# DavidSlayback/po-brax

Measured on AMD Instinct MI355X. Metric: env-steps/sec AntHeavenHell batch 65536 @1/2/4/8 GPU; % HBM roofline, higher is better.
Workload: dtype f32

## Files before the change

### po-brax_amd/csrc/pob_blockwalk.h

```cpp
#pragma once
#include <stdint.h>
#ifdef POB_BW_HOST
#define POB_BW_D static inline
#else
#define POB_BW_D __device__ __forceinline__
#endif

#define QBW_WAVES 4
#define QBW_WCAP 50
#define QBW_SLOT_DW 11
#define QBW_CON_DW 5
#define QBW_LANE_MAX 64
#define QBW_CAP (QBW_WAVES * QBW_WCAP)
#define QBW_SEG_FLOATS (QBW_WCAP * QBW_SLOT_DW + 1)
#define QBW_NO_CONTACT (-1)

POB_BW_D constexpr int bw_item_off(const int j) { return QBW_SLOT_DW * j; }
POB_BW_D constexpr int bw_meta_off(const int j) { return QBW_SLOT_DW * j + 2 * QBW_CON_DW; }
POB_BW_D constexpr int bw_con_off(const int c) { return QBW_SLOT_DW * (c >> 1) + QBW_CON_DW * (c & 1); }
POB_BW_D constexpr int bw_count_off() { return QBW_WCAP * QBW_SLOT_DW; }

POB_BW_D constexpr int bw_meta(const int bit, const bool seg, const int slot) { return bit | (seg ? 64 : 0) | (slot << 7); }
POB_BW_D constexpr int bw_meta_bit(const int m) { return m & 63; }
POB_BW_D constexpr bool bw_meta_seg(const int m) { return (m & 64) != 0; }
POB_BW_D constexpr int bw_meta_slot(const int m) { return (m >> 7) & 3; }

POB_BW_D int bw_lane_count(const uint64_t m0, const uint64_t m1, const uint64_t m2) {
  const int n = __builtin_popcountll(m0) + __builtin_popcountll(m1) + __builtin_popcountll(m2);
  return n < QBW_LANE_MAX ? n : QBW_LANE_MAX;
}
POB_BW_D void bw_prefix_step(const uint64_t m, const int lane, const int b, int &base, int &tot) {
  base += __builtin_popcountll(m & ((1ull << lane) - 1ull)) << b;
  tot += __builtin_popcountll(m) << b;
}
#define QBW_PREFIX_BITS 7
#define QBW_PREFIX_SHORT_BITS 2
POB_BW_D constexpr bool bw_prefix_needs_all(const int count) { return count >= (1 << QBW_PREFIX_SHORT_BITS); }

POB_BW_D bool bw_next_item(uint64_t (&M)[3], int &slot, int &bit) {
  const bool h0 = M[0] != 0ull, h1 = M[1] != 0ull, h2 = M[2] != 0ull;
  const bool has = h0 | h1 | h2;
  slot = h0 ? 0 : (h1 ? 1 : 2);
  const uint64_t ml = h0 ? M[0] : (h1 ? M[1] : M[2]);
  bit = has ? __builtin_ctzll(ml) : 0;
  const uint64_t pop = has ? ml & (0ull - ml) : 0ull;
  M[0] = h0 ? M[0] & ~pop : M[0];
  M[1] = (!h0 & h1) ? M[1] & ~pop : M[1];
  M[2] = (!h0 & !h1) ? M[2] & ~pop : M[2];
  return has;
}

struct BwDeal {
  int off[QBW_WAVES];
  int T;
  bool ovf;
};
POB_BW_D BwDeal bw_deal(const int n0, const int n1, const int n2, const int n3, const int cap) {
  BwDeal d;
  d.off[0] = 0; d.off[1] = n0; d.off[2] = n0 + n1; d.off[3] = n0 + n1 + n2;
  const int T = n0 + n1 + n2 + n3;
  d.ovf = (T > cap) | (n0 > QBW_WCAP) | (n1 > QBW_WCAP) | (n2 > QBW_WCAP) | (n3 > QBW_WCAP);
  d.T = d.ovf ? 0 : T;
  return d;
}
POB_BW_D int bw_rounds(const BwDeal &d) { return (d.T + 7) >> 3; }
POB_BW_D int bw_first_round(const int w, const int sub) { return (w + sub) & (QBW_WAVES - 1); }
POB_BW_D void bw_item_owner(const BwDeal &d, const int i, int &w, int &j) {
  w = (i >= d.off[1] ? 1 : 0) + (i >= d.off[2] ? 1 : 0) + (i >= d.off[3] ? 1 : 0);
  j = i - (w == 0 ? 0 : (w == 1 ? d.off[1] : (w == 2 ? d.off[2] : d.off[3])));
}
POB_BW_D void bw_apply_range(const int base, const int n, const bool ovf, int &c0, int &c1) {
  c0 = 2 * base;
  c1 = ovf ? c0 : 2 * (base + n);
}
POB_BW_D void bw_body_ranges(const int base, const int n0, const int n1, const int n2, const bool ovf, int (&c)[4]) {
  c[0] = 2 * base;
  c[1] = ovf ? c[0] : c[0] + 2 * n0;
  c[2] = ovf ? c[0] : c[1] + 2 * n1;
  c[3] = ovf ? c[0] : c[2] + 2 * n2;
}

POB_BW_D constexpr bool bw_quad_lead(const int lane) { return (lane & 3) == 0; }
POB_BW_D constexpr int bw_quad_torso_count(const int lane, const int n0) { return bw_quad_lead(lane) ? n0 : 0; }
POB_BW_D void bw_quad_ranges(const int lane, const int base0, const int n0, const int base, const int n1, const int n2,
                             const bool ovf, int (&c)[5]) {
  c[0] = 2 * base0;
  c[1] = ovf ? c[0] : c[0] + 2 * n0;
  c[2] = 2 * (base + bw_quad_torso_count(lane, n0));
  c[3] = ovf ? c[2] : c[2] + 2 * n1;
  c[4] = ovf ? c[2] : c[3] + 2 * n2;
}

#define QBW_HIT_ITEMS 16
POB_BW_D constexpr uint32_t bw_hit_bits(const bool h0, const bool h1, const int i) {
  return ((h0 ? 1u : 0u) | (h1 ? 2u : 0u)) << (2 * i);
}
POB_BW_D constexpr int bw_hit_count(const int tot, const bool wide) { return wide && tot <= QBW_WCAP ? QBW_WCAP + 1 : tot; }
```

### po-brax_amd/csrc/pob_kernels.hip

```cpp
#include <hip/hip_fp16.h>
#include <hip/hip_runtime.h>

#include <climits>
#include <cstdio>
#include <cstdlib>
#include <cstring>
#include <mutex>
#include <new>
#include <type_traits>
#include <vector>

#include "../../include/pob.h"

#include "pob_quad.h"
#include "pob_octet.h"
#include "pob_hexa.h"
#include "pob_physics.h"

namespace pob {
void default_params(pob_params &p);
const char *build_system(int kind, const pob_params &p, pob_sys &s);
int gather_grid(const pob_params &p, float *xyz, int cap);
}

struct pob_env {
  pob_sys sys;
  pob_sys *d_sys = nullptr;
  pob_params params;
  float *d_grid = nullptr;
  uint32_t *d_scratch = nullptr;
  int device = 0;
  int n_cu = 256;
};

#define POB_MIXED (-1)
#define POB_F_STAGED (1u << 16)
#define POB_F_INT_FORCE_FIXUP (1u << 30)
#define POB_F_INT_BWCAP_SHIFT 20
#define POB_F_INT_BWCAP_MASK (0xFFu << POB_F_INT_BWCAP_SHIFT)
#define POB_F_INT_HITW_SHIFT 17
#define POB_F_INT_HITW_MASK (0x7u << POB_F_INT_HITW_SHIFT)
#define POB_F_INTERNAL (POB_F_STAGED | POB_F_INT_FORCE_FIXUP | POB_F_INT_BWCAP_MASK | POB_F_INT_HITW_MASK)
#define POB_F_PUBLIC (POB_F_EPISODE | POB_F_AUTORESET | POB_F_ZERO_STEPS_ON_DONE)

#define POB_STATE_FIELDS(X)                                                                    \
  X(pos) X(rot) X(vel) X(ang) X(obs) X(reward) X(done) X(steps) X(truncation) X(m0) X(m1) X(m2) \
  X(rng) X(first_pos) X(first_rot) X(first_vel) X(first_ang) X(first_obs) X(any_done) X(done_u8) X(trunc_i32) \
  X(m0_i32) X(m1_i32) X(any_done_clear) X(obs_masked) X(ovf_mark)

struct StatePtrs {
  float *pos, *rot, *vel, *ang, *obs, *reward, *done, *steps, *truncation, *m0, *m1, *m2;
  uint32_t *rng;
  float *first_pos, *first_rot, *first_vel, *first_ang, *first_obs;
  uint32_t *any_done;
  uint8_t *done_u8;
  int32_t *trunc_i32, *m0_i32, *m1_i32;
  uint32_t *any_done_clear;
  float *obs_masked;
  uint8_t *ovf_mark;
};
POB_D void store_obs_masked(csys_t &S, float *dst, const float *stg, const int rows, const int D, const int lane) {
  const int K = S.obs_mask_n;
  for (int r = 0; r < rows; ++r)
    for (int c = lane; c < K; c += 64) dst[(size_t)r * K + c] = stg[r * D + S.obs_mask[c]];
}
static StatePtrs to_ptrs(const pob_state &s) {
  StatePtrs p;
#define POB_CP(f) p.f = s.f;
  POB_STATE_FIELDS(POB_CP)
#undef POB_CP
  return p;
}

template <typename QT> struct Q;
template <> struct Q<float> {
  static POB_D float ld(const float *p, size_t i) { return p[i]; }
  static POB_D void st(float *p, size_t i, float v) { p[i] = v; }
};
template <> struct Q<__half> {
  static POB_D float ld(const float *p, size_t i) { return __half2float(reinterpret_cast<const __half *>(p)[i]); }
  static POB_D void st(float *p, size_t i, float v) {
    asm volatile("" : "+v"(v));
    reinterpret_cast<__half *>(p)[i] = __float2half_rn(v);
  }
};
template <typename QT> POB_D v3 ld3(const float *p, size_t i) {
  return V(Q<QT>::ld(p, i), Q<QT>::ld(p, i + 1), Q<QT>::ld(p, i + 2));
}
template <typename QT> POB_D void st3(float *p, size_t i, v3 v) {
  Q<QT>::st(p, i, v.x); Q<QT>::st(p, i + 1, v.y); Q<QT>::st(p, i + 2, v.z);
}
template <typename QT> POB_D q4 ld4(const float *p, size_t i) {
  q4 q; q.w = Q<QT>::ld(p, i); q.x = Q<QT>::ld(p, i + 1); q.y = Q<QT>::ld(p, i + 2); q.z = Q<QT>::ld(p, i + 3);
  return q;
}
template <typename QT> POB_D void st4(float *p, size_t i, q4 q) {
  Q<QT>::st(p, i, q.w); Q<QT>::st(p, i + 1, q.x); Q<QT>::st(p, i + 2, q.y); Q<QT>::st(p, i + 3, q.z);
}
template <typename QT> POB_D void cpq(float *dst, const float *src, size_t i, int n) {
  for (int k = 0; k < n; ++k) Q<QT>::st(dst, i + k, Q<QT>::ld(src, i + k));
}
template <typename QT, int L, int U>
POB_D void group_cpq(float *dst, const float *src, const size_t i, const int n, const int j) {
  for (int q0 = j; q0 < n; q0 += L * U) {
    float v[U];
#pragma unroll
    for (int u = 0; u < U; ++u) v[u] = q0 + L * u < n ? Q<QT>::ld(src, i + q0 + L * u) : 0.0f;
#pragma unroll
    for (int u = 0; u < U; ++u)
      if (q0 + L * u < n) Q<QT>::st(dst, i + q0 + L * u, v[u]);
  }
}
template <int L, int U>
POB_D void group_copy(float *dst, const float *src, const int n, const int j) {
  for (int q0 = j; q0 < n; q0 += L * U) {
    float v[U];
#pragma unroll
    for (int u = 0; u < U; ++u) v[u] = q0 + L * u < n ? src[q0 + L * u] : 0.0f;
#pragma unroll
    for (int u = 0; u < U; ++u)
      if (q0 + L * u < n) dst[q0 + L * u] = v[u];
  }
}
template <typename QT, int L, int U = 4>
POB_D void tail_copies(const StatePtrs &in, const StatePtrs &out, const uint32_t flags, const bool reset_rows,
// ... 401 lines not shown
#pragma unroll
        for (int q = 0; q < 3; ++q)
          if (q < n_el - i) stg[i + q] = v[m][q];
      }
    }
  }
};

template <typename QT, int C>
POB_D void stage_store_dyn(float *X, size_t el0, int N, int nenv, const float *stg, int lane) {
  constexpr int C9 = POB_NDYN * C;
  if (sizeof(QT) == 4 && (C == 3 || (reinterpret_cast<uintptr_t>(X) & 15) == 0)) {
    struct alignas(4) f3 { float a, b, c; };
    for (int r = lane; r < nenv * POB_NDYN; r += 64) {
      const int e = r / POB_NDYN, g = r - e * POB_NDYN;
      float *dst = X + el0 + (size_t)e * N * C + g * C;
      const float *src = stg + r * C;
      if constexpr (C == 4) *reinterpret_cast<float4 *>(dst) = *reinterpret_cast<const float4 *>(src);
      else *reinterpret_cast<f3 *>(dst) = f3{src[0], src[1], src[2]};
    }
  } else {
    for (int i = lane; i < nenv * C9; i += 64) {
      const int e = i / C9, j = i - e * C9;
      Q<QT>::st(X, el0 + (size_t)e * N * C + j, stg[i]);
    }
  }
}

template <int N>
POB_D void stage_table(float *dst, const __attribute__((address_space(4))) float *src, const int tid,
                       const int stride) {
  constexpr int M = (N + 63) / 64;
  float v[M];
#pragma unroll
  for (int m = 0; m < M; ++m) {
    const int i = tid + stride * m;
    v[m] = i < N ? src[i] : 0.0f;
  }
#pragma unroll
  for (int m = 0; m < M; ++m) {
    const int i = tid + stride * m;
    if (i < N) dst[i] = v[m];
  }
}
POB_D void stage_leg_table(csys_t *Sp, float *legtab) {
  const __attribute__((address_space(4))) float *src = &Sp->leg[0][0];
  stage_table<POB_TAB_FLOATS>(legtab, src, (int)threadIdx.x, (int)blockDim.x);
  __syncthreads();
}
#ifdef POB_EXP_TIMING
#define POB_TS_WAVES 65536
#ifdef POB_EXP_TIMING_SUB
#define POB_TS_N 16
#else
#define POB_TS_N 10
#endif
#define POB_TS_ROW (POB_TS_N + 4)
__device__ unsigned long long pob_ts_buf[POB_TS_WAVES * POB_TS_ROW];
#define POB_TS_DECL() \
  unsigned long long pob_ts[POB_TS_N] = {}; \
  const unsigned long long pob_rt0 = __builtin_amdgcn_s_memrealtime()
#define POB_TS(i) pob_ts[i] = __builtin_amdgcn_s_memtime()
#define POB_TS_WRITE()                                                                   \
  do {                                                                                   \
    POB_TS(POB_TS_N - 1);                                                                \
    if ((threadIdx.x & 63) == 0) {                                                       \
      unsigned hwid, xcc;                                                                \
      asm volatile("s_getreg_b32 %0, hwreg(HW_REG_HW_ID)" : "=s"(hwid));                 \
      asm volatile("s_getreg_b32 %0, hwreg(HW_REG_XCC_ID)" : "=s"(xcc));                 \
      const size_t w = (size_t)blockIdx.x * (blockDim.x >> 6) + (threadIdx.x >> 6);      \
      if (w < POB_TS_WAVES) {                                                            \
        unsigned long long *r = pob_ts_buf + w * POB_TS_ROW;                             \
        r[0] = hwid; r[1] = xcc;                                                         \
        for (int i = 0; i < POB_TS_N; ++i) r[2 + i] = pob_ts[i];                         \
        r[POB_TS_N + 2] = pob_rt0; r[POB_TS_N + 3] = __builtin_amdgcn_s_memrealtime();    \
      }                                                                                  \
    }                                                                                    \
  } while (0)
#else
#define POB_TS_DECL() ((void)0)
#define POB_TS(i) ((void)0)
#define POB_TS_WRITE() ((void)0)
#endif
template <typename QT>
__device__ __forceinline__ void quad_store_dyn(const StatePtrs &in, const StatePtrs &out, const QBody &bd,
                                               const bool act_lane, const int k, const int le, const int b_first,
                                               const int nenv, const int N, const size_t r3, const size_t r4,
                                               float *stg, const int lane, const bool reset_rows) {
#pragma unroll
  for (int arr = 0; arr < 4; ++arr) {
    const int c = arr == 1 ? 4 : 3;
    if (act_lane) {
#pragma unroll
      for (int l = 0; l < QNB; ++l) {
        if (l == 0 && k != 0) continue;
        const int g = qbody_global(l, k);
        float *o = stg + (le * POB_NDYN + g) * c;
        if (reset_rows) {
          const float *F = arr == 0 ? in.first_pos : (arr == 1 ? in.first_rot : (arr == 2 ? in.first_vel : in.first_ang));
          const size_t src = (arr == 1 ? r4 : r3) + (size_t)g * c;
          for (int q = 0; q < c; ++q) o[q] = Q<QT>::ld(F, src + q);
        } else if (arr == 0) { o[0] = bd.x[l].x; o[1] = bd.x[l].y; o[2] = bd.x[l].z; }
        else if (arr == 1) { o[0] = bd.q[l].w; o[1] = bd.q[l].x; o[2] = bd.q[l].y; o[3] = bd.q[l].z; }
        else if (arr == 2) { o[0] = bd.v[l].x; o[1] = bd.v[l].y; o[2] = bd.v[l].z; }
        else { o[0] = bd.w[l].x; o[1] = bd.w[l].y; o[2] = bd.w[l].z; }
      }
    }
    wave_lds_sync();
    if (arr == 1) stage_store_dyn<QT, 4>(out.rot, (size_t)b_first * N * 4, N, nenv, stg, lane);
    else stage_store_dyn<QT, 3>(arr == 0 ? out.pos : (arr == 2 ? out.vel : out.ang), (size_t)b_first * N * 3, N,
                                nenv, stg, lane);
    wave_lds_sync();
  }
}

template <int KIND, typename QT>
__device__ __attribute__((noinline)) void quad_fixup(const void *kargs, int gt, uint32_t stg_at, uint32_t lds_at,
                                                     uint32_t legtab_at);
POB_D void substep_prio(const int it, const int iters) {
  const int lvl = (it * 4) / (2 * iters);
  if (lvl == 0) __builtin_amdgcn_s_setprio(3);
  else if (lvl == 1) __builtin_amdgcn_s_setprio(2);
  else if (lvl == 2) __builtin_amdgcn_s_setprio(1);
  else __builtin_amdgcn_s_setprio(0);
}
typedef __attribute__((address_space(3))) float lds_float;
POB_D uint32_t lds_addr(const float *p) { return (uint32_t)(size_t)(const lds_float *)p; }
POB_D float *lds_ptr(const uint32_t at) { return (float *)(lds_float *)(size_t)at; }
template <int KIND, typename QT, bool LEG = false, int MODE = 0, bool COOP = false>
POB_D void step_quad_body(csys_t *Sp, const int B, const StatePtrs &in, const float *__restrict__ act,
                          const StatePtrs &out, const uint32_t flags, const int L, const int gt, const int tid,
                          float *lds, const float *legtab) {
  csys_t &S = *Sp;
  const int lane = tid & 63;
  POB_TS_DECL();
  POB_TS(0);
  float *stg = lds + (tid >> 6) * POB_STAGE_FLOATS;
  const QLds Ls{stg, lane};
  int b = gt >> 2;
  int k = gt & 3;
  const float *LT = legtab + k * POB_LEG_FLOATS;
  const float *WT = legtab + 4 * POB_LEG_FLOATS;
  const int kind = KIND != POB_MIXED ? KIND : S.kind;
  const int N = n_bodies<KIND>(S), D = obs_dim<KIND>(S);
  const int sh = obs_shift(kind);
  bool act_lane = b < B;
  int b_first = (gt - lane) >> 2;
  const bool dead = b_first >= B;
  if (!COOP && dead) return;
  if (MODE == 2 && out.ovf_mark[b_first] == 0) return;
  if (MODE == 1 && lane == 0 && !dead) out.ovf_mark[b_first] = 0;
  if (COOP && dead) b_first = ((B - 1) >> 4) << 4;
  int nenv = B - b_first < 16 ? B - b_first : 16;
  int le = b - b_first;
  int bl = act_lane ? b : B - 1, lel = bl - b_first;
  size_t r3 = (size_t)bl * N * 3, r4 = (size_t)bl * N * 4;
  constexpr bool FUSED = MODE == 1 && COOP;
  auto fixup = [&]() {
    if constexpr (FUSED)
      quad_fixup<KIND, QT>((const void *)__builtin_amdgcn_kernarg_segment_ptr(), gt, lds_addr(stg), lds_addr(lds),
                           lds_addr(legtab));
  };
  auto rederive = [&]() {
    int g2 = gt;
    asm volatile("" : "+v"(g2));
    b = g2 >> 2;
    k = g2 & 3;
    act_lane = b < B;
    b_first = (g2 - (g2 & 63)) >> 2;
    nenv = B - b_first < 16 ? B - b_first : 16;
    le = b - b_first;
    bl = act_lane ? b : B - 1;
    lel = bl - b_first;
    r3 = (size_t)bl * N * 3;
    r4 = (size_t)bl * N * 4;
  };

  QBody bd;
  constexpr int NMAX = KIND == POB_HEAVENHELL ? 14 : (KIND == POB_TAG ? 12 : (KIND == POB_ANT ? 10 : POB_MAXB));
  constexpr int MAXI = (16 * NMAX * 4 + 255) / 256;
  if ((flags & POB_F_STAGED) && NMAX <= 16 && N == NMAX && 16 * N * 7 <= POB_STAGE_FLOATS) {
#pragma unroll
    for (int pr = 0; pr < 2; ++pr) {
      const int c0 = 3, c1 = pr == 0 ? 4 : 3;
      const int n0 = nenv * N * c0, n1 = nenv * N * c1;
      ChunkLoad<QT, MAXI> A0, A1;
      A0.template issue<NMAX * 3, POB_NDYN * 3>(pr == 0 ? in.pos : in.vel, (size_t)b_first * N * c0, n0, lane);
      if (pr == 0) A1.template issue<NMAX * 4, POB_NDYN * 4>(in.rot, (size_t)b_first * N * c1, n1, lane);
      else A1.template issue<NMAX * 3, POB_NDYN * 3>(in.ang, (size_t)b_first * N * c1, n1, lane);
      A0.template put<NMAX * 3, POB_NDYN * 3>(stg, n0, lane);
      if (pr == 0) A1.template put<NMAX * 4, POB_NDYN * 4>(stg + n0, n1, lane);
      else A1.template put<NMAX * 3, POB_NDYN * 3>(stg + n0, n1, lane);
      wave_lds_sync();
      {
#pragma unroll
        for (int l = 0; l < QNB; ++l) {
          const int g = qbody_global(l, k);
          const float *s0 = stg + (lel * N + g) * c0, *s1 = stg + n0 + (lel * N + g) * c1;
          if (pr == 0) {
            bd.x[l] = V(s0[0], s0[1], s0[2]);
            bd.q[l].w = s1[0]; bd.q[l].x = s1[1]; bd.q[l].y = s1[2]; bd.q[l].z = s1[3];
          } else {
            bd.v[l] = V(s0[0], s0[1], s0[2]);
            bd.w[l] = V(s1[0], s1[1], s1[2]);
          }
        }
      }
      wave_lds_sync();
    }
  } else if (flags & POB_F_STAGED) {
#pragma unroll
    for (int arr = 0; arr < 4; ++arr) {
      const int c = arr == 1 ? 4 : 3;
      const float *X = arr == 0 ? in.pos : (arr == 1 ? in.rot : (arr == 2 ? in.vel : in.ang));
      stage_load<QT>(X, (size_t)b_first * N * c, nenv * N * c, stg, lane);
      wave_lds_sync();
      {
#pragma unroll
        for (int l = 0; l < QNB; ++l) {
          const int o = (lel * N + qbody_global(l, k)) * c;
          if (arr == 0) bd.x[l] = V(stg[o], stg[o + 1], stg[o + 2]);
          else if (arr == 1) { bd.q[l].w = stg[o]; bd.q[l].x = stg[o + 1]; bd.q[l].y = stg[o + 2]; bd.q[l].z = stg[o + 3]; }
          else if (arr == 2) bd.v[l] = V(stg[o], stg[o + 1], stg[o + 2]);
          else bd.w[l] = V(stg[o], stg[o + 1], stg[o + 2]);
        }
      }
      wave_lds_sync();
    }
  } else {
#pragma unroll
    for (int l = 0; l < QNB; ++l) {
      const int g = qbody_global(l, k);
      bd.x[l] = ld3<QT>(in.pos, r3 + 3 * g);
      bd.q[l] = ld4<QT>(in.rot, r4 + 4 * g);
      bd.v[l] = ld3<QT>(in.vel, r3 + 3 * g);
      bd.w[l] = ld3<QT>(in.ang, r3 + 3 * g);
    }
  }

  POB_TS(1);
#define POB_QUAD_NEAR_MARGIN 0.5f
  float jang[QNJ], jvel[QNJ];
  v3 cvl[QNB], cal[QNB];
  TaskOut t;
  t.tp_ok = false;
  {
    float a[QNJ];
#pragma unroll
    for (int jl = 0; jl < QNJ; ++jl) a[jl] = act[(size_t)bl * POB_NJ + 2 * k + jl];
#pragma unroll
    for (int l = 0; l < QNB; ++l) { Ls.set3(l, QF_CV, V(0.0f, 0.0f, 0.0f)); Ls.set3(l, QF_CA, V(0.0f, 0.0f, 0.0f)); }
    const int iters = Sp->substeps / 2;
    const float fric = quad_friction(S);
#define POB_QUAD_FAST_PASS 4
#define POB_QUAD_REDERIVE 22
    constexpr int KBIT = KIND < 0 ? 16 : 1 << KIND;
    constexpr bool FASTP = (POB_QUAD_FAST_PASS & KBIT) != 0, REDER = (POB_QUAD_REDERIVE & KBIT) != 0;
    if (LEG) {
#pragma nounroll
      for (int it = 0; it < Sp->substeps; ++it) qlegacy_substep<KIND != POB_ANT>(Sp, LT, WT, bd, a, Ls);
    } else {
    constexpr bool TWO = KIND == POB_GATHER;
    constexpr bool WALLS = KIND != POB_ANT;
    int pass = TWO ? (__any(qwall_mask_margin(S, bd, POB_QUAD_NEAR_MARGIN) != 0u) ? 1 : 0) : 1;
    auto reload = [&]() {
#pragma unroll
      for (int l = 0; l < QNB; ++l) {
        const int g = qbody_global(l, k);
        bd.x[l] = ld3<QT>(in.pos, r3 + 3 * g);
        bd.q[l] = ld4<QT>(in.rot, r4 + 4 * g);
        bd.v[l] = ld3<QT>(in.vel, r3 + 3 * g);
        bd.w[l] = ld3<QT>(in.ang, r3 + 3 * g);
        Ls.set3(l, QF_CV, V(0.0f, 0.0f, 0.0f));
        Ls.set3(l, QF_CA, V(0.0f, 0.0f, 0.0f));
      }
    };
    for (;;) {
    if (pass == 0) {
      bool near = false;
#pragma nounroll
      for (int it = 0; it < 2 * iters; ++it) {
        substep_prio(it, iters);
        qpbd_substep<false, true>(Sp, LT, WT, bd, a, Ls, (it & 1) != 0, fric, &near);
      }
      if (!__any(near)) break;
      pass = 1;
      reload();
      continue;
    }
    if constexpr (MODE == 1 && WALLS && COOP) {
      const int capf = (int)((flags & POB_F_INT_BWCAP_MASK) >> POB_F_INT_BWCAP_SHIFT);
      const int hitf = (int)((flags & POB_F_INT_HITW_MASK) >> POB_F_INT_HITW_SHIFT);
      QBlock blk{lds + QPOOL_OFF, __builtin_amdgcn_readfirstlane(tid >> 6), 0,
                 capf != 0 ? capf : QBW_CAP, hitf != 0 ? hitf : QBW_HIT_ITEMS, dead, false};
#pragma nounroll
      for (int it = 0; it < 2 * iters; ++it) {
        substep_prio(it, iters);
        qpbd_substep<WALLS, false, false, true>(Sp, LT, WT, bd, a, Ls, (it & 1) != 0, fric, nullptr, nullptr, &blk);
      }
      if (dead) return;
      if (__builtin_expect(blk.ovf || (flags & POB_F_INT_FORCE_FIXUP), 0)) {
        if (lane == 0) out.ovf_mark[b_first] = 1;
        fixup();
        return;
      }
      break;
    }
    if (MODE == 1 && WALLS) {
      bool ovf = false;
#pragma nounroll
      for (int it = 0; it < 2 * iters; ++it) {
        substep_prio(it, iters);
        qpbd_substep<WALLS, false, false>(Sp, LT, WT, bd, a, Ls, (it & 1) != 0, fric, nullptr, &ovf);
        if (__any(ovf)) break;
      }
      if (__builtin_expect(__any(ovf) || (flags & POB_F_INT_FORCE_FIXUP), 0)) {
        if (lane == 0) out.ovf_mark[b_first] = 1;
        fixup();
        return;
      }
      break;
    }
    if (pass == 1 && WALLS && FASTP && MODE == 0) {
      bool ovf = false;
#pragma nounroll
      for (int it = 0; it < 2 * iters; ++it) {
        substep_prio(it, iters);
        qpbd_substep<WALLS, false, false>(Sp, LT, WT, bd, a, Ls, (it & 1) != 0, fric, nullptr, &ovf);
        if (__any(ovf)) break;
      }
      if (!__any(ovf)) break;
      pass = 2;
      reload();
      continue;
    }
#pragma nounroll
    for (int it = 0; it < 2 * iters; ++it) {
      substep_prio(it, iters);
      if (WALLS && FASTP && MODE == 0) {
        QSlow st;
        st.b = bd;
#pragma unroll
        for (int j = 0; j < QNJ; ++j) st.act[j] = a[j];
        qpbd_substep_slow<WALLS>(Sp, LT, WT, &st, Ls.base, Ls.t, (it & 1) != 0 ? 1 : 0, fric);
        bd = st.b;
      } else
      qpbd_substep<WALLS>(Sp, LT, WT, bd, a, Ls, (it & 1) != 0, fric);
    }
    break;
    }
    }
    if constexpr (REDER) rederive();
    const float xb = ld3<QT>(in.pos, r3).x;
#pragma unroll
    for (int jl = 0; jl < QNJ; ++jl) {
      const int p = jparent(jl), c = jchild(jl);
      v3 ap = qrot(QJV(LT, jl, QJ_AXIS), bd.q[p]);
      const v3 ref = jl == 0 ? V(-1.0f, 0.0f, 0.0f) : V(0.0f, 0.0f, 1.0f);
      v3 fp = qrot(ref, bd.q[p]), fc = qrot(ref, bd.q[c]);
      jang[jl] = pob_atan2f(vdot(vcross(fp, fc), ap), vdot(fp, fc));
      jvel[jl] = vdot(vsub(bd.w[c], bd.w[p]), ap);
    }
#pragma unroll
    for (int l = 0; l < QNB; ++l) { cvl[l] = Ls.get3(l, QF_CV); cal[l] = Ls.get3(l, QF_CA); }
    if (act_lane && k == 0) {
      float steps = in.steps ? in.steps[b] : 0.0f;
      if ((flags & (POB_F_AUTORESET | POB_F_ZERO_STEPS_ON_DONE)) && in.done[b] != 0.0f) steps = 0.0f;
      t.steps = steps;
      t.m0 = in.m0 ? in.m0[b] : 0.0f; t.m1 = in.m1 ? in.m1[b] : 0.0f; t.m2 = in.m2 ? in.m2[b] : 0.0f;
      t.rng0 = in.rng[2 * b]; t.rng1 = in.rng[2 * b + 1];
      t.xb = xb; t.ctrl = 0.0f; t.contact = 0.0f;
      if (kind == POB_ANT) {
        t.ctrl = ant_ctrl_cost(act + (size_t)b * POB_NJ);
        float sc = 0.0f;
#pragma unroll
        for (int l = 0; l < QNB; ++l) sc = ant_contact_add(sc, cvl[l]);
#pragma unroll
        for (int q = 1; q < 4; ++q) {
#pragma unroll
          for (int l = 1; l < QNB; ++l) sc = ant_contact_add(sc, Ls.get3_lane(l, QF_CV, lane + q));
        }
        t.contact = 0.0005f * sc;
      }
    }
  }
  wave_lds_sync();
  POB_TS(2);

  float done = 0.0f;
  t.ga_done_quad = false;
  const bool ga_quad = (KIND == POB_GATHER || KIND == POB_MIXED) && kind == POB_GATHER && S.n_obj <= POB_GA_QUAD_MAX;
  GaQuad gq;
  if (ga_quad && act_lane) {
    v3 gop[4];
    ga_quad_prefetch<QT>(S, in, r3, nullptr, k, gop);
    ga_quad_objects<QT>(S, gop, r3, bd.x[0], bd.q[0], k, out.pos, gq, t);
  }
#ifdef POB_EXP_TIMING_OBS
  POB_TS(3);
#endif
  const bool task_in_pass = kind == POB_GATHER && !ga_quad;
  if (act_lane && k == 0 && out.pos != in.pos) {
    for (int i = POB_NDYN; i < N; ++i) {
      if (!(ga_quad && i >= 11)) cpq<QT>(out.pos, in.pos, r3 + 3 * i, 3);
      cpq<QT>(out.vel, in.vel, r3 + 3 * i, 3);
      cpq<QT>(out.ang, in.ang, r3 + 3 * i, 3);
      cpq<QT>(out.rot, in.rot, r4 + 4 * i, 4);
    }
  }
  if (!task_in_pass && act_lane) {
    if (k == 0) {
      task_dispatch<KIND, QT>(S, kind, in, b, r3, N, bd.x[0], bd.q[0], out.pos, nullptr, flags, L, t);
      done = t.done;
    }
    done = quad_bcast<0>(done);
  }
#ifdef POB_EXP_TIMING_OBS
  POB_TS(4);
#endif
  const int P = pass_envs(POB_STAGE_FLOATS, D, 16);
  for (int p0 = 0; p0 < nenv; p0 += P) {
    const int pn = nenv - p0 < P ? nenv - p0 : P;
    if (act_lane && le >= p0 && le < p0 + pn) {
      float *o = stg + (le - p0) * D;
#pragma unroll
      for (int jl = 0; jl < QNJ; ++jl) {
        o[sh + 7 + 2 * k + jl] = jang[jl];
        o[sh + 21 + 2 * k + jl] = jvel[jl];
      }
      float *oc = o + (29 + sh);
#pragma unroll
      for (int l = 0; l < QNB; ++l) {
        if (l == 0 && k != 0) continue;
        const int g = qbody_global(l, k);
        oc[3 * g] = clip1(cvl[l].x); oc[1 + 3 * g] = clip1(cvl[l].y); oc[2 + 3 * g] = clip1(cvl[l].z);
        oc[3 * N + 3 * g] = clip1(cal[l].x); oc[1 + 3 * N + 3 * g] = clip1(cal[l].y); oc[2 + 3 * N + 3 * g] = clip1(cal[l].z);
      }
      for (int q = 3 * POB_NDYN + k; q < 3 * N; q += 4) { oc[q] = 0.0f; oc[3 * N + q] = 0.0f; }
      if (k == 0) {
        if (sh == 0) { o[0] = bd.x[0].x; o[1] = bd.x[0].y; }
        o[sh + 2] = bd.x[0].z;
        o[sh + 3] = bd.q[0].w; o[sh + 4] = bd.q[0].x; o[sh + 5] = bd.q[0].y; o[sh + 6] = bd.q[0].z;
        o[sh + 15] = bd.v[0].x; o[sh + 16] = bd.v[0].y; o[sh + 17] = bd.v[0].z;
        o[sh + 18] = bd.w[0].x; o[sh + 19] = bd.w[0].y; o[sh + 20] = bd.w[0].z;
      }
      if (ga_quad) ga_quad_scatter(S, gq, k, o + 29 + 6 * N);
      if (task_in_pass) {
        if (k == 0) {
          task_dispatch<KIND, QT>(S, kind, in, b, r3, N, bd.x[0], bd.q[0], out.pos, o, flags, L, t);
          done = t.done;
        }
        done = quad_bcast<0>(done);
      } else if (k == 0) {
        task_obs_write(kind, o, 29 + 6 * N, t);
      }
      if ((flags & POB_F_AUTORESET) && done != 0.0f) {
        wave_lds_sync();
        group_copy<4, 4>(o, in.first_obs + (size_t)b * D, D, k);
      }
    }
#ifdef POB_EXP_TIMING_OBS
    if (p0 == 0) POB_TS(5);
#endif
    wave_lds_sync();
    float *dst = out.obs + (size_t)(b_first + p0) * D;
    const int n = pn * D;
    if ((reinterpret_cast<uintptr_t>(dst) & 15) == 0) {
      const int n4 = n >> 2;
      for (int i = lane; i < n4; i += 64) reinterpret_cast<float4 *>(dst)[i] = reinterpret_cast<const float4 *>(stg)[i];
      for (int i = 4 * n4 + lane; i < n; i += 64) dst[i] = stg[i];
    } else {
      for (int i = lane; i < n; i += 64) dst[i] = stg[i];
    }
    if (out.obs_masked)
      store_obs_masked(S, out.obs_masked + (size_t)(b_first + p0) * S.obs_mask_n, stg, pn, D, lane);
    wave_lds_sync();
#ifdef POB_EXP_TIMING_OBS
    if (p0 == 0) POB_TS(6);
#endif
  }

#ifdef POB_EXP_TIMING_OBS
  POB_TS(7);
#else
  POB_TS(3);
#endif
  const bool reset_rows = (flags & POB_F_AUTORESET) && done != 0.0f;
  quad_store_dyn<QT>(in, out, bd, act_lane, k, le, b_first, nenv, N, r3, r4, stg, lane, reset_rows);
#ifdef POB_EXP_TIMING_OBS
  POB_TS(8);
#else
  POB_TS(4);
#endif
  if (act_lane) tail_copies<QT, 4, 2>(in, out, flags, reset_rows, b, N, D, r3, r4, k);
  if (act_lane && k == 0) {
    out.reward[b] = t.reward;
    out.done[b] = t.done;
    if (out.steps) out.steps[b] = t.steps;
    if (out.truncation) out.truncation[b] = t.trunc;
    if (out.m0) out.m0[b] = t.m0;
    if (out.m1) out.m1[b] = t.m1;
    if (out.m2) out.m2[b] = t.m2;
    out.rng[2 * b] = t.rng0;
    out.rng[2 * b + 1] = t.rng1;
    write_typed(out, b, t);
  }
  if (out.any_done) {
    const unsigned long long m = __ballot(act_lane && k == 0 && done != 0.0f);
    if (m != 0ull && lane == 0) atomicOr(out.any_done, 1u);
  }
  POB_TS_WRITE();
}

POB_D bool quad_block_marked(const int B, const uint8_t *mark, const int bt0) {
  bool any = false;
  for (int w = 0; w < (int)blockDim.x / 64; ++w) {
    const int bf = (bt0 + 64 * w) >> 2;
    if (bf < B) any = any | (mark[bf] != 0);
  }
  return any;
}
template <int KIND, typename QT, int MODE = 0, bool COOP = false>
__global__ __launch_bounds__(256, POB_QUAD_MIN_WAVES) void k_step_quad(const void *sysp, const int B,
                                                                       const StatePtrs in,
                                                                       const float *__restrict__ act,
                                                                       const StatePtrs out, const uint32_t flags,
                                                                       const int L) {
  static_assert(MODE <= 2, "MODE 3 is quad_fixup's");
  static_assert(!COOP || (MODE == 1 && (KIND == POB_HEAVENHELL || KIND == POB_TAG)), "the cooperative walk: fast pass, HH / TAG");
  __shared__ __attribute__((aligned(16))) float lds[QL_FLOATS * 256];
  __shared__ __attribute__((aligned(16))) float legtab[POB_TAB_FLOATS];
  if (MODE == 2 && !quad_block_marked(B, out.ovf_mark, (int)(blockIdx.x * blockDim.x)))
    return;
  stage_leg_table((csys_t *)(size_t)sysp, legtab);
  step_quad_body<KIND, QT, false, MODE, COOP>((csys_t *)(size_t)sysp, B, in, act, out, flags, L,
                                        (int)(blockIdx.x * blockDim.x + threadIdx.x), (int)threadIdx.x, lds, legtab);
}

template <typename QT>
__global__ __launch_bounds__(256, 3) void k_step_quad_ga3(const void *sysp, const int B, const StatePtrs in,
                                                          const float *__restrict__ act, const StatePtrs out,
                                                          const uint32_t flags, const int L) {
  __shared__ float lds[QL_FLOATS * 256];
  __shared__ __attribute__((aligned(16))) float legtab[POB_TAB_FLOATS];
  stage_leg_table((csys_t *)(size_t)sysp, legtab);
  step_quad_body<POB_GATHER, QT>((csys_t *)(size_t)sysp, B, in, act, out, flags, L,
                                 (int)(blockIdx.x * blockDim.x + threadIdx.x), (int)threadIdx.x, lds, legtab);
}

template <int KIND, typename QT>
__global__ __launch_bounds__(256) void k_step_legacy(const void *sysp, const int B, const StatePtrs in,
                                                     const float *__restrict__ act, const StatePtrs out,
                                                     const uint32_t flags, const int L) {
  __shared__ float lds[QL_FLOATS * 256];
  __shared__ __attribute__((aligned(16))) float legtab[POB_TAB_FLOATS];
  stage_leg_table((csys_t *)(size_t)sysp, legtab);
  step_quad_body<KIND, QT, true>((csys_t *)(size_t)sysp, B, in, act, out, flags, L,
                                 (int)(blockIdx.x * blockDim.x + threadIdx.x), (int)threadIdx.x, lds, legtab);
}

struct MixSeg {
  const void *sysp;
  const float *act;
  StatePtrs in, out;
  int B, blk0;
};
struct MixArgs {
  MixSeg s[POB_MIX_MAX];
  int n;
};
static_assert(POB_MIX_MAX == 4, "pick_state selects among 4 segments");
// ... 1344 lines not shown
    case POB_HEAVENHELL: hipLaunchKernelGGL((k_reset<POB_HEAVENHELL, 64, QT>), g, dim3(64), shm, st, sp, B, mode, keys, gin, gout, flag, p, total, first, WP); break;
    case POB_GATHER: hipLaunchKernelGGL((k_reset<POB_GATHER, 64, QT>), g, dim3(64), shm, st, sp, B, mode, keys, gin, gout, flag, p, total, first, WP); break;
    case POB_TAG: hipLaunchKernelGGL((k_reset<POB_TAG, 64, QT>), g, dim3(64), shm, st, sp, B, mode, keys, gin, gout, flag, p, total, first, WP); break;
    default: hipLaunchKernelGGL((k_reset<POB_ANT, 64, QT>), g, dim3(64), shm, st, sp, B, mode, keys, gin, gout, flag, p, total, first, WP); break;
  }
}
static int octet_max_batch() {
  const char *e = getenv("POB_OCTET_MAX_B");
  return e ? atoi(e) : 16384;
}
static int hexa_max_batch(int n_cu, int kind) {
  const char *e = getenv("POB_HEXA_MAX_B");
  if (e) return atoi(e);
  return (kind == POB_HEAVENHELL || kind == POB_TAG ? 32 : 16) * n_cu;
}
template <typename QT, bool GACC>
static void launch_step_hex_g(int kind, hipStream_t st, const void *sp, int B, const StatePtrs &pi, const float *act,
                              const StatePtrs &po, uint32_t flags, int L, int n_cu) {
  const dim3 g((unsigned)((B + 3) / 4)), b(64);
  if ((B + 3) / 4 > 4 * n_cu) {
    if (kind == POB_HEAVENHELL) {
      hipLaunchKernelGGL((k_step_hex<POB_HEAVENHELL, QT, GACC, true>), g, b, 0, st, sp, B, pi, act, po, flags, L);
      return;
    }
    if (kind == POB_TAG) {
      hipLaunchKernelGGL((k_step_hex<POB_TAG, QT, GACC, true>), g, b, 0, st, sp, B, pi, act, po, flags, L);
      return;
    }
  }
  switch (kind) {
    case POB_HEAVENHELL: hipLaunchKernelGGL((k_step_hex<POB_HEAVENHELL, QT, GACC>), g, b, 0, st, sp, B, pi, act, po, flags, L); break;
    case POB_GATHER: hipLaunchKernelGGL((k_step_hex<POB_GATHER, QT, GACC>), g, b, 0, st, sp, B, pi, act, po, flags, L); break;
    case POB_TAG: hipLaunchKernelGGL((k_step_hex<POB_TAG, QT, GACC>), g, b, 0, st, sp, B, pi, act, po, flags, L); break;
    default: hipLaunchKernelGGL((k_step_hex<POB_ANT, QT, GACC>), g, b, 0, st, sp, B, pi, act, po, flags, L); break;
  }
}
template <typename QT>
static void launch_step_hex(int kind, int n_cu, hipStream_t st, const void *sp, int B, const StatePtrs &pi,
                            const float *act, const StatePtrs &po, uint32_t flags, int L) {
  const char *f = getenv("POB_HEX_GACC");
  const bool acc = f ? atoi(f) != 0 : (kind == POB_HEAVENHELL || kind == POB_TAG || (B + 3) / 4 <= 4 * n_cu);
  if (acc) launch_step_hex_g<QT, true>(kind, st, sp, B, pi, act, po, flags, L, n_cu);
  else launch_step_hex_g<QT, false>(kind, st, sp, B, pi, act, po, flags, L, n_cu);
}
template <typename QT, bool GACC>
static void launch_step_oct_g(int kind, hipStream_t st, const void *sp, int B, const StatePtrs &pi, const float *act,
                              const StatePtrs &po, uint32_t flags, int L) {
  const dim3 g((unsigned)((B + 7) / 8)), b(64);
  switch (kind) {
    case POB_HEAVENHELL: hipLaunchKernelGGL((k_step_oct<POB_HEAVENHELL, QT, GACC>), g, b, 0, st, sp, B, pi, act, po, flags, L); break;
    case POB_GATHER: hipLaunchKernelGGL((k_step_oct<POB_GATHER, QT, GACC>), g, b, 0, st, sp, B, pi, act, po, flags, L); break;
    case POB_TAG: hipLaunchKernelGGL((k_step_oct<POB_TAG, QT, GACC>), g, b, 0, st, sp, B, pi, act, po, flags, L); break;
    default: hipLaunchKernelGGL((k_step_oct<POB_ANT, QT, GACC>), g, b, 0, st, sp, B, pi, act, po, flags, L); break;
  }
}
template <typename QT>
static void launch_step_oct(int kind, int n_cu, hipStream_t st, const void *sp, int B, const StatePtrs &pi,
                            const float *act, const StatePtrs &po, uint32_t flags, int L) {
  const char *f = getenv("POB_OCT_GACC");
  const bool acc = f ? atoi(f) != 0 : (B + 7) / 8 <= 4 * n_cu;
  if (acc) launch_step_oct_g<QT, true>(kind, st, sp, B, pi, act, po, flags, L);
  else launch_step_oct_g<QT, false>(kind, st, sp, B, pi, act, po, flags, L);
}
#define POB_QUAD_SPLIT_KINDS 23
static bool quad_split_launch(int kind) {
  const char *f = getenv("POB_QUAD_SPLIT");
  if (f) return atoi(f) != 0;
  return ((POB_QUAD_SPLIT_KINDS >> (kind < 0 ? 4 : kind)) & 1) != 0;
}
static uint32_t quad_force_fixup() {
  const char *f = getenv("POB_QUAD_FORCE_FIXUP");
  return f && atoi(f) != 0 ? POB_F_INT_FORCE_FIXUP : 0u;
}
static uint32_t quad_block_cap() {
  const char *f = getenv("POB_QUAD_BLOCK_CAP");
  const int n = f ? atoi(f) : 0;
  return n >= 1 && n < QBW_CAP ? (uint32_t)n << POB_F_INT_BWCAP_SHIFT : 0u;
}
static uint32_t quad_hit_width() {
  const char *f = getenv("POB_QUAD_HIT_WIDTH");
  const int n = f ? atoi(f) : 0;
  return n >= 1 && n <= 7 ? (uint32_t)n << POB_F_INT_HITW_SHIFT : 0u;
}
template <typename QT>
static void launch_step_quad(int kind, bool legacy, int n_cu, hipStream_t st, const void *sp, int B,
                             const StatePtrs &pi, const float *act, const StatePtrs &po, uint32_t flags, int L) {
  const int bs = 4 * B <= 64 * 256 ? 64 : 256;
  const dim3 g = grid_for(4 * B, bs), b(bs);
  if (legacy) {
    switch (kind) {
      case POB_HEAVENHELL: hipLaunchKernelGGL((k_step_legacy<POB_HEAVENHELL, QT>), g, b, 0, st, sp, B, pi, act, po, flags, L); break;
      case POB_GATHER: hipLaunchKernelGGL((k_step_legacy<POB_GATHER, QT>), g, b, 0, st, sp, B, pi, act, po, flags, L); break;
      case POB_TAG: hipLaunchKernelGGL((k_step_legacy<POB_TAG, QT>), g, b, 0, st, sp, B, pi, act, po, flags, L); break;
      default: hipLaunchKernelGGL((k_step_legacy<POB_ANT, QT>), g, b, 0, st, sp, B, pi, act, po, flags, L); break;
    }
    return;
  }
  if (kind == POB_GATHER && (size_t)4 * B <= (size_t)3 * 64 * 4 * n_cu) {
    hipLaunchKernelGGL((k_step_quad_ga3<QT>), g, b, 0, st, sp, B, pi, act, po, flags, L);
    return;
  }
  const bool split = quad_split_launch(kind) && po.ovf_mark != nullptr;
  flags |= split ? quad_force_fixup() : 0u;
  const bool coop = split && bs == 256 && (kind == POB_HEAVENHELL || kind == POB_TAG);
  flags |= coop ? quad_block_cap() | quad_hit_width() : 0u;
  const bool second = split && !coop;
  switch (kind) {
    case POB_HEAVENHELL:
      if (split) {
        if (coop) hipLaunchKernelGGL((k_step_quad<POB_HEAVENHELL, QT, 1, true>), g, b, 0, st, sp, B, pi, act, po, flags, L);
        else hipLaunchKernelGGL((k_step_quad<POB_HEAVENHELL, QT, 1>), g, b, 0, st, sp, B, pi, act, po, flags, L);
        if (second) hipLaunchKernelGGL((k_step_quad<POB_HEAVENHELL, QT, 2>), g, b, 0, st, sp, B, pi, act, po, flags, L);
      } else {
        hipLaunchKernelGGL((k_step_quad<POB_HEAVENHELL, QT>), g, b, 0, st, sp, B, pi, act, po, flags, L);
      }
      break;
    case POB_GATHER:
      if (split) {
        hipLaunchKernelGGL((k_step_quad<POB_GATHER, QT, 1>), g, b, 0, st, sp, B, pi, act, po, flags, L);
        if (second) hipLaunchKernelGGL((k_step_quad<POB_GATHER, QT, 2>), g, b, 0, st, sp, B, pi, act, po, flags, L);
      } else {
        hipLaunchKernelGGL((k_step_quad<POB_GATHER, QT>), g, b, 0, st, sp, B, pi, act, po, flags, L);
      }
      break;
    case POB_TAG:
      if (split) {
        if (coop) hipLaunchKernelGGL((k_step_quad<POB_TAG, QT, 1, true>), g, b, 0, st, sp, B, pi, act, po, flags, L);
        else hipLaunchKernelGGL((k_step_quad<POB_TAG, QT, 1>), g, b, 0, st, sp, B, pi, act, po, flags, L);
        if (second) hipLaunchKernelGGL((k_step_quad<POB_TAG, QT, 2>), g, b, 0, st, sp, B, pi, act, po, flags, L);
      } else {
        hipLaunchKernelGGL((k_step_quad<POB_TAG, QT>), g, b, 0, st, sp, B, pi, act, po, flags, L);
      }
      break;
    default: hipLaunchKernelGGL((k_step_quad<POB_ANT, QT>), g, b, 0, st, sp, B, pi, act, po, flags, L); break;
  }
}
extern "C" {

int pob_abi_version(void) { return POB_ABI_VERSION; }
const char *pob_last_error(void) { return g_err; }

int pob_default_params(pob_params *p) {
  if (!p) return fail(POB_EINVAL, "params is NULL");
  pob::default_params(*p);
  return POB_OK;
}

static std::mutex g_grave_mu;
static std::vector<void *> g_grave;

static void drain_grave() {
  std::vector<void *> dead;
  {
    std::lock_guard<std::mutex> lk(g_grave_mu);
    dead.swap(g_grave);
  }
  for (void *p : dead) (void)hipFree(p);
}

int pob_env_create(int kind, const pob_params *p, pob_env **out) {
  if (!out) return fail(POB_EINVAL, "out is NULL");
  *out = nullptr;
  drain_grave();
  pob_params prm;
  if (p) prm = *p; else pob::default_params(prm);
  pob_env *e = new (std::nothrow) pob_env();
  if (!e) return fail(POB_ENOMEM, "out of host memory");
  e->params = prm;
  if (const char *msg = pob::build_system(kind, prm, e->sys)) { delete e; return fail(POB_EINVAL, msg); }
  int rc = hip_check(hipGetDevice(&e->device), "hipGetDevice");
  if (!rc) rc = hip_check(hipDeviceGetAttribute(&e->n_cu, hipDeviceAttributeMultiprocessorCount, e->device),
                          "hipDeviceGetAttribute(CUs)");
  if (rc) { delete e; return rc; }
  rc = hip_check(hipMalloc(&e->d_scratch, 64), "hipMalloc(scratch)");
  if (rc) { delete e; return rc; }
  if (kind == POB_GATHER) {
    static float tmp[3 * 4096];
    const int n = pob::gather_grid(prm, tmp, 4096);
    rc = hip_check(hipMalloc(&e->d_grid, sizeof(float) * 3 * n), "hipMalloc(grid)");
    if (!rc) rc = hip_check(hipMemcpy(e->d_grid, tmp, sizeof(float) * 3 * n, hipMemcpyHostToDevice), "hipMemcpy(grid)");
    if (rc) { (void)hipFree(e->d_scratch); delete e; return rc; }
    e->sys.grid = e->d_grid;
  }
  rc = hip_check(hipMalloc(&e->d_sys, sizeof(pob_sys)), "hipMalloc(sys)");
  if (!rc) rc = hip_check(hipMemcpy(e->d_sys, &e->sys, sizeof(pob_sys), hipMemcpyHostToDevice), "hipMemcpy(sys)");
  if (rc) { if (e->d_grid) (void)hipFree(e->d_grid); (void)hipFree(e->d_scratch); delete e; return rc; }
  *out = e;
  return POB_OK;
// ... 274 lines not shown
```

Measured before the change: 550.8 million.

## Deal near-wall environments evenly across waves in cooperative quad step

Adds a block-level step that balances environments across waves in the cooperative HeavenHell quad kernel. Each block takes a ballot of which environments are near walls, shares the packed masks through LDS, and reassigns environment slots so near-wall (expensive) environments are spread evenly over the four waves. Staging and stores then go through block-wide barriers and per-wave LDS regions chosen by slot instead of wave-local syncs. The aim is to reduce wave divergence and load imbalance in the contact path, at the cost of extra block barriers, select/popcount arithmetic and more complex indexing.

```diff
diff --git a/po-brax_amd/csrc/pob_blockwalk.h b/po-brax_amd/csrc/pob_blockwalk.h
--- a/po-brax_amd/csrc/pob_blockwalk.h
+++ b/po-brax_amd/csrc/pob_blockwalk.h
@@ -91,6 +91,46 @@
   c[4] = ovf ? c[2] : c[3] + 2 * n2;
 }
 
+POB_BW_D int bw_div_small(const int n, const int k) {
+  return k == 1 ? n : (k == 2 ? n >> 1 : (k == 3 ? (n * 43) >> 7 : n >> 2));
+}
+POB_BW_D int bw_select64(uint64_t m, int r) {
+  int pos = 0;
+  for (int w = 32; w >= 1; w >>= 1) {
+    const int c = __builtin_popcountll(m & ((1ull << w) - 1ull));
+    const bool up = r >= c;
+    r -= up ? c : 0;
+    m = up ? m >> w : m;
+    pos += up ? w : 0;
+  }
+  return pos;
+}
+POB_BW_D int bw_deal_waves(const int n, const int cap) {
+  const int k = (n + cap - 1) / cap;
+  return k > QBW_WAVES ? QBW_WAVES : k;
+}
+POB_BW_D int bw_deal_count(const int n, const int k, const int j) {
+  return j < k ? bw_div_small(n + k - 1 - j, k) : 0;
+}
+POB_BW_D int bw_env_deal(const uint64_t near, const int blk, const int cap, const int w, const int q) {
+  const int n = __builtin_popcountll(near);
+  const int k = bw_deal_waves(n, cap);
+  const int j = (w - blk) & (QBW_WAVES - 1);
+  const int cj = bw_deal_count(n, k, j);
+  if (q < cj) return bw_select64(near, q * k + j);
+  int f = q - cj;
+  for (int i = 0; i < QBW_WAVES - 1; ++i) f += i < j ? 16 - bw_deal_count(n, k, i) : 0;
+  return bw_select64(~near, f);
+}
+POB_BW_D uint32_t bw_pack_quads(uint64_t x) {
+  x &= 0x1111111111111111ull;
+  x = (x | (x >> 3)) & 0x0303030303030303ull;
+  x = (x | (x >> 6)) & 0x000F000F000F000Full;
+  x = (x | (x >> 12)) & 0x000000FF000000FFull;
+  x = (x | (x >> 24)) & 0xFFFFull;
+  return (uint32_t)x;
+}
+
 #define QBW_HIT_ITEMS 16
 POB_BW_D constexpr uint32_t bw_hit_bits(const bool h0, const bool h1, const int i) {
   return ((h0 ? 1u : 0u) | (h1 ? 2u : 0u)) << (2 * i);
diff --git a/po-brax_amd/csrc/pob_kernels.hip b/po-brax_amd/csrc/pob_kernels.hip
--- a/po-brax_amd/csrc/pob_kernels.hip
+++ b/po-brax_amd/csrc/pob_kernels.hip
@@ -40,7 +40,9 @@
 #define POB_F_INT_BWCAP_MASK (0xFFu << POB_F_INT_BWCAP_SHIFT)
 #define POB_F_INT_HITW_SHIFT 17
 #define POB_F_INT_HITW_MASK (0x7u << POB_F_INT_HITW_SHIFT)
-#define POB_F_INTERNAL (POB_F_STAGED | POB_F_INT_FORCE_FIXUP | POB_F_INT_BWCAP_MASK | POB_F_INT_HITW_MASK)
+#define POB_F_INT_DEAL (1u << 28)
+#define POB_F_INT_DEAL_NOROT (1u << 29)
+#define POB_F_INTERNAL (POB_F_STAGED | POB_F_INT_FORCE_FIXUP | POB_F_INT_BWCAP_MASK | POB_F_INT_HITW_MASK | POB_F_INT_DEAL | POB_F_INT_DEAL_NOROT)
 #define POB_F_PUBLIC (POB_F_EPISODE | POB_F_AUTORESET | POB_F_ZERO_STEPS_ON_DONE)
 
 #define POB_STATE_FIELDS(X)                                                                    \
@@ -608,11 +610,17 @@
 #define POB_TS(i) ((void)0)
 #define POB_TS_WRITE() ((void)0)
 #endif
+POB_D void region_sync(const bool dealt) {
+  if (dealt) qblock_barrier();
+  else wave_lds_sync();
+}
 template <typename QT>
 __device__ __forceinline__ void quad_store_dyn(const StatePtrs &in, const StatePtrs &out, const QBody &bd,
                                                const bool act_lane, const int k, const int le, const int b_first,
                                                const int nenv, const int N, const size_t r3, const size_t r4,
-                                               float *stg, const int lane, const bool reset_rows) {
+                                               float *stg, const int lane, const bool reset_rows,
+                                               float *stg_h = nullptr, const bool dealt = false) {
+  if (!dealt) stg_h = stg;
 #pragma unroll
   for (int arr = 0; arr < 4; ++arr) {
     const int c = arr == 1 ? 4 : 3;
@@ -621,7 +629,7 @@
       for (int l = 0; l < QNB; ++l) {
         if (l == 0 && k != 0) continue;
         const int g = qbody_global(l, k);
-        float *o = stg + (le * POB_NDYN + g) * c;
+        float *o = stg_h + (le * POB_NDYN + g) * c;
         if (reset_rows) {
           const float *F = arr == 0 ? in.first_pos : (arr == 1 ? in.first_rot : (arr == 2 ? in.first_vel : in.first_ang));
           const size_t src = (arr == 1 ? r4 : r3) + (size_t)g * c;
@@ -632,11 +640,11 @@
         else { o[0] = bd.w[l].x; o[1] = bd.w[l].y; o[2] = bd.w[l].z; }
       }
     }
-    wave_lds_sync();
+    region_sync(dealt);
     if (arr == 1) stage_store_dyn<QT, 4>(out.rot, (size_t)b_first * N * 4, N, nenv, stg, lane);
     else stage_store_dyn<QT, 3>(arr == 0 ? out.pos : (arr == 2 ? out.vel : out.ang), (size_t)b_first * N * 3, N,
                                 nenv, stg, lane);
-    wave_lds_sync();
+    region_sync(dealt);
   }
 }
 
@@ -687,15 +695,57 @@
       quad_fixup<KIND, QT>((const void *)__builtin_amdgcn_kernarg_segment_ptr(), gt, lds_addr(stg), lds_addr(lds),
                            lds_addr(legtab));
   };
+#define POB_QUAD_DEAL_MARGIN (-0.05f)
+#define POB_QUAD_DEAL_CAP 14
+  constexpr bool DEAL = MODE == 1 && COOP;
+  int slot = (tid >> 2) & 63;
+  bool dealt = false;
+  const float *hs = stg;
+  const bool deal_on = DEAL && (flags & POB_F_INT_DEAL) != 0 && !(flags & POB_F_INT_FORCE_FIXUP) &&
+                       ((gt - tid) >> 2) + 64 <= B &&
+                       N == (KIND == POB_HEAVENHELL ? 14 : 12);
+  auto deal = [&](const v3 (&nx)[QNB]) {
+    QBody nb;
+#pragma unroll
+    for (int l = 0; l < QNB; ++l) nb.x[l] = nx[l];
+    uint64_t bal = __ballot(qwall_mask_margin(S, nb, POB_QUAD_DEAL_MARGIN) != 0u);
+    bal |= bal >> 1;
+    bal |= bal >> 2;
+    float *xw = lds + (POB_STAGE_FLOATS - 1);
+    if (lane == 0) xw[(tid >> 6) * POB_STAGE_FLOATS] = __int_as_float((int)bw_pack_quads(bal));
+    qblock_barrier();
+    uint64_t near = 0ull;
+#pragma unroll
+    for (int w = 0; w < QBW_WAVES; ++w)
+      near |= (uint64_t)(uint32_t)__builtin_amdgcn_readfirstlane(__float_as_int(xw[w * POB_STAGE_FLOATS])) << (16 * w);
+    const int n = __builtin_popcountll(near);
+    dealt = n != 0 && n != 64;
+    if (dealt) {
+      slot = bw_env_deal(near, (flags & POB_F_INT_DEAL_NOROT) ? 0 : (gt - tid) >> 8, POB_QUAD_DEAL_CAP, tid >> 6, lane >> 2);
+      hs = lds + (slot >> 4) * POB_STAGE_FLOATS;
+      b = ((gt - tid) >> 2) + slot;
+      bl = b;
+      lel = slot & 15;
+      r3 = (size_t)bl * N * 3;
+      r4 = (size_t)bl * N * 4;
+    }
+  };
+  static_assert(QBW_SEG_FLOATS + QPOOL_OFF < POB_STAGE_FLOATS, "the near-mask word lies past the exchange segment");
   auto rederive = [&]() {
     int g2 = gt;
     asm volatile("" : "+v"(g2));
     b = g2 >> 2;
     k = g2 & 3;
+    b_first = (g2 - (g2 & 63)) >> 2;
+    if constexpr (DEAL) {
+      const int sw = __float_as_int(*(stg + 64 * QLL_HEAD + (g2 & 63)));
+      slot = sw & 63;
+      dealt = __builtin_amdgcn_readfirstlane(sw >> 6) != 0;
+      b = ((g2 - (g2 & 255)) >> 2) + slot;
+    }
     act_lane = b < B;
-    b_first = (g2 - (g2 & 63)) >> 2;
     nenv = B - b_first < 16 ? B - b_first : 16;
-    le = b - b_first;
+    le = DEAL ? slot & 15 : b - b_first;
     bl = act_lane ? b : B - 1;
     lel = bl - b_first;
     r3 = (size_t)bl * N * 3;
@@ -717,12 +767,23 @@
       A0.template put<NMAX * 3, POB_NDYN * 3>(stg, n0, lane);
       if (pr == 0) A1.template put<NMAX * 4, POB_NDYN * 4>(stg + n0, n1, lane);
       else A1.template put<NMAX * 3, POB_NDYN * 3>(stg + n0, n1, lane);
-      wave_lds_sync();
+      if (DEAL && pr == 0 && deal_on) {
+        wave_lds_sync();
+        v3 nx[QNB];
+#pragma unroll
+        for (int l = 0; l < QNB; ++l) {
+          const float *s0 = stg + (lel * N + qbody_global(l, k)) * c0;
+          nx[l] = V(s0[0], s0[1], s0[2]);
+        }
+        deal(nx);
+      } else {
+        region_sync(dealt);
+      }
       {
 #pragma unroll
         for (int l = 0; l < QNB; ++l) {
           const int g = qbody_global(l, k);
-          const float *s0 = stg + (lel * N + g) * c0, *s1 = stg + n0 + (lel * N + g) * c1;
+          const float *s0 = hs + (lel * N + g) * c0, *s1 = hs + n0 + (lel * N + g) * c1;
           if (pr == 0) {
             bd.x[l] = V(s0[0], s0[1], s0[2]);
             bd.q[l].w = s1[0]; bd.q[l].x = s1[1]; bd.q[l].y = s1[2]; bd.q[l].z = s1[3];
@@ -732,7 +793,7 @@
           }
         }
       }
-      wave_lds_sync();
+      region_sync(dealt);
     }
   } else if (flags & POB_F_STAGED) {
 #pragma unroll
@@ -754,6 +815,12 @@
       wave_lds_sync();
     }
   } else {
+    if (DEAL && deal_on) {
+      v3 nx[QNB];
+#pragma unroll
+      for (int l = 0; l < QNB; ++l) nx[l] = ld3<QT>(in.pos, r3 + 3 * qbody_global(l, k));
+      deal(nx);
+    }
 #pragma unroll
     for (int l = 0; l < QNB; ++l) {
       const int g = qbody_global(l, k);
@@ -763,6 +830,7 @@
       bd.w[l] = ld3<QT>(in.ang, r3 + 3 * g);
     }
   }
+  if constexpr (DEAL) *Ls.head() = __int_as_float(slot | (dealt ? 64 : 0));
 
   POB_TS(1);
 #define POB_QUAD_NEAR_MARGIN 0.5f
@@ -876,7 +944,7 @@
     break;
     }
     }
-    if constexpr (REDER) rederive();
+    if constexpr (REDER || DEAL) rederive();
     const float xb = ld3<QT>(in.pos, r3).x;
 #pragma unroll
     for (int jl = 0; jl < QNJ; ++jl) {
@@ -910,7 +978,8 @@
       }
     }
   }
-  wave_lds_sync();
+  region_sync(dealt);
+  float *stg_h = DEAL && dealt ? lds + (slot >> 4) * POB_STAGE_FLOATS : stg;
   POB_TS(2);
 
   float done = 0.0f;
@@ -948,7 +1017,7 @@
   for (int p0 = 0; p0 < nenv; p0 += P) {
     const int pn = nenv - p0 < P ? nenv - p0 : P;
     if (act_lane && le >= p0 && le < p0 + pn) {
-      float *o = stg + (le - p0) * D;
+      float *o = stg_h + (le - p0) * D;
 #pragma unroll
       for (int jl = 0; jl < QNJ; ++jl) {
         o[sh + 7 + 2 * k + jl] = jang[jl];
@@ -988,7 +1057,7 @@
 #ifdef POB_EXP_TIMING_OBS
     if (p0 == 0) POB_TS(5);
 #endif
-    wave_lds_sync();
+    region_sync(dealt);
     float *dst = out.obs + (size_t)(b_first + p0) * D;
     const int n = pn * D;
     if ((reinterpret_cast<uintptr_t>(dst) & 15) == 0) {
@@ -1000,7 +1069,7 @@
     }
     if (out.obs_masked)
       store_obs_masked(S, out.obs_masked + (size_t)(b_first + p0) * S.obs_mask_n, stg, pn, D, lane);
-    wave_lds_sync();
+    region_sync(dealt);
 #ifdef POB_EXP_TIMING_OBS
     if (p0 == 0) POB_TS(6);
 #endif
@@ -1012,7 +1081,7 @@
   POB_TS(3);
 #endif
   const bool reset_rows = (flags & POB_F_AUTORESET) && done != 0.0f;
-  quad_store_dyn<QT>(in, out, bd, act_lane, k, le, b_first, nenv, N, r3, r4, stg, lane, reset_rows);
+  quad_store_dyn<QT>(in, out, bd, act_lane, k, le, b_first, nenv, N, r3, r4, stg, lane, reset_rows, stg_h, DEAL && dealt);
 #ifdef POB_EXP_TIMING_OBS
   POB_TS(8);
 #else
@@ -2523,10 +2592,16 @@
   const int n = f ? atoi(f) : 0;
   return n >= 1 && n <= 7 ? (uint32_t)n << POB_F_INT_HITW_SHIFT : 0u;
 }
+static uint32_t quad_deal(const int kind, const uint32_t hooks) {
+  const char *f = getenv("POB_QUAD_DEAL");
+  if (f) return atoi(f) == 0 ? 0u : (atoi(f) == 2 ? POB_F_INT_DEAL | POB_F_INT_DEAL_NOROT : POB_F_INT_DEAL);
+  return kind == POB_HEAVENHELL && hooks == 0u ? POB_F_INT_DEAL : 0u;
+}
 template <typename QT>
 static void launch_step_quad(int kind, bool legacy, int n_cu, hipStream_t st, const void *sp, int B,
                              const StatePtrs &pi, const float *act, const StatePtrs &po, uint32_t flags, int L) {
-  const int bs = 4 * B <= 64 * 256 ? 64 : 256;
+  const char *bt = getenv("POB_QUAD_BLOCK_THREADS");
+  const int bs = bt && atoi(bt) == 256 ? 256 : (4 * B <= 64 * 256 ? 64 : 256);
   const dim3 g = grid_for(4 * B, bs), b(bs);
   if (legacy) {
     switch (kind) {
@@ -2545,6 +2620,7 @@
   flags |= split ? quad_force_fixup() : 0u;
   const bool coop = split && bs == 256 && (kind == POB_HEAVENHELL || kind == POB_TAG);
   flags |= coop ? quad_block_cap() | quad_hit_width() : 0u;
+  flags |= coop ? quad_deal(kind, flags & (POB_F_INT_BWCAP_MASK | POB_F_INT_HITW_MASK)) : 0u;
   const bool second = split && !coop;
   switch (kind) {
     case POB_HEAVENHELL:
```

After: 549.8 million. About the same (-0.2%).
